# hmc-lair-shark-tracking/auv-sim

Hardware: AMD Instinct MI355X
Metric: RRT-Dubins node expansions/s (RRT.exploring) (higher is better)
Workload: dtype f64; 1 GPU; RRT.exploring 256 obst 200x200 cells 10000 iters x 12288 episodes/GPU, timebin parent sampling; episodes_per_gpu=12288, iters=10000, obstacles=256, cells=40000, parallelism=episodes sharded x1

## Files before the change

### auv_sim_amd/csrc/rrt_rows_body.h

```cpp
  extern __shared__ __align__(16) unsigned char smem[];
  const RrtTables S = rrt_tables_view(smem, W.n_habitats, W.n_poly);
  const int wave = (int)(threadIdx.x >> 6);
  const int lane = lane_id();
  const int row = lane >> 4, rl = lane & 15, rowbase = lane & 48;
  const int K = P.K;
  const int wg_waves = (int)(blockDim.x >> 6);
#if AUVP_ROWS_BODY_STREAM
  const RowsStreamLdsPlan plan = rrt_rows_stream_lds_plan(K, RW_MAX_OBST, rrt_tables_bytes(W.n_habitats, W.n_poly, W.n_bins), wg_waves, MIRROR);
  unsigned char* ebase = smem + plan.tables + (size_t)(wave * RW_ROWS + row) * plan.per_ep;
  double* ring = reinterpret_cast<double*>(ebase);
  double* inc = reinterpret_cast<double*>(ebase + plan.ring);
  uint16_t* bin_count = reinterpret_cast<uint16_t*>(ebase + plan.ring + plan.scratch);
#else
  const RowsLdsPlan plan = rrt_rows_lds_plan(K, RW_MAX_OBST, rrt_tables_bytes(W.n_habitats, W.n_poly, W.n_bins), wg_waves);
  unsigned char* ebase = smem + plan.tables + (size_t)(wave * RW_ROWS + row) * plan.per_ep;
  uint32_t* mt = reinterpret_cast<uint32_t*>(ebase);
  double* win = reinterpret_cast<double*>(ebase + plan.mt);
  double* inc = win;
  uint16_t* bin_count = reinterpret_cast<uint16_t*>(ebase + plan.mt + plan.scratch);
#endif

  rrt_tables_stage(S, W);
  if (threadIdx.x == 0) *S.params = P;
  const RrtParamsDev& Q = *S.params;
  double* olx = reinterpret_cast<double*>(smem + plan.tables + (size_t)wg_waves * RW_ROWS * plan.per_ep);
  double* oly = olx + RW_MAX_OBST;
  float* olr = reinterpret_cast<float*>(oly + RW_MAX_OBST);
  for (int i = threadIdx.x; i < RW_MAX_OBST; i += blockDim.x) { olx[i] = W.os_x[i]; oly[i] = W.os_y[i]; olr[i] = W.os_r[i]; }
  __syncthreads();

  const int ep = ((int)blockIdx.x * wg_waves + wave) * RW_ROWS + row;
  bool live = ep < n_episodes;
  const int eps = live ? ep : 0;
  if (!wave_any(live)) return;

  const int capn = B.cap_nodes, capp = B.cap_points, bcap = B.bin_cap;
  double* nodeF = B.node_f + (size_t)eps * capn * 8;
  int4* nodeI = reinterpret_cast<int4*>(B.node_i) + (size_t)eps * capn;
  uint8_t* nodeQ = B.node_q + (size_t)eps * capn;
  double* ptF = B.points + (size_t)eps * capp * 6;
  const BinLists bins = bin_lists(B, (size_t)eps, K);
  int next_chunk = 0;
  const double* init = B.init + (size_t)eps * 6;

#if AUVP_ROWS_BODY_STREAM
  RowStream rng;
  rng.ring = ring;
  rng.src = B.stream + (size_t)eps * (size_t)B.stream_cap;
  rng.pos = 0u; rng.front = 0u; rng.req = 0u;
  rng.cap = (uint32_t)B.stream_cap;
#pragma unroll
  for (int c = 0; c < RS_PEND; c++) rng.pend[c] = rs_piece(0.0);
#ifdef AUVP_STREAM_COUNT_SLOW
  rng.slow = 0u;
#endif
#define ROWS_CONSUME(on, n) stream_advance(rng, on, (uint32_t)(n))
#else
  RowRng rng;
  rng.s = mt;
  for (int i = rl; i < 624; i += 16) mt[i] = B.mt[(size_t)eps * 624 + i];
  {
    int idx = B.mt_index ? B.mt_index[eps] : 624;
    idx = idx < 0 ? 0 : (idx > 624 ? 624 : idx);
    rng.pslot = idx == 624 ? 0u : (uint32_t)idx;
    rng.avail = (uint32_t)(624 - idx);
    rng.drawn = 0ull;
  }
#define ROWS_CONSUME(on, n) rows_advance(rng, on, (uint32_t)(2 * (n)))
#endif
  for (int i = rl; i < K + 2; i += 16) bin_count[i] = 0;
  wave_sync();
  if (live && rl == 0) {
    nodeF[0] = init[0]; nodeF[1] = init[1]; nodeF[2] = init[2]; nodeF[3] = init[3]; nodeF[4] = init[5];
    nodeI[0] = make_int4(0, -1, 0, 0);
    nodeQ[0] = 0;
    bins.direct[(K >= 1 ? 1 : 0) * AUVP_BIN_HEAD] = 0;
    bin_count[K >= 1 ? 1 : 0] = 1;
  }
  wave_sync();
  int n_nodes = 1, n_points = 0, status = 0, n_cand = 0, iters_run = 0;
  const double4 sbox = reinterpret_cast<const double4*>(W.os_box)[rl];
  const int nv_poly = W.n_poly;

  for (int it = 0; it < P.max_iter; it++) {
    if (!wave_any(live)) break;
    int par = 0, n_total = 0, base = 0;
    {
      bool search = live;
      int fo = 0, rb = 0, cnt = 0;
      double u = 0.0;
#if AUVP_ROWS_BODY_STREAM
      StreamBase<MIRROR> sel;
#endif
      for (;;) {
#if AUVP_ROWS_BODY_STREAM
        if (!stream_ensure<MIRROR>(rng, search, 16u, rl) && search) { status = AUVP_ST_STREAM; live = false; iters_run = it; search = false; }
        sel = stream_base<MIRROR>(rng, 0u, rl);
        if (search) u = stream_read(sel, rl, rl);
#else
        rows_ensure(rng, search, 32u, rl);
        if (search) { u = rows_random_at(rng, (uint32_t)rl); win[rl] = u; }
#endif
        const int rbj = (int)py_uniform(1.0, (double)(K + 1), u);
        const bool cand = search && rl < 14;
        const bool badkey = cand && rbj > K;
        const int cj = (cand && !badkey) ? (int)bin_count[rbj] : 0;
        const uint32_t okm = row_ballot(cj != 0, rowbase), badm = row_ballot(badkey, rowbase);
        const int f_ok = okm ? (__ffs((int)okm) - 1) : 16, f_bad = badm ? (__ffs((int)badm) - 1) : 16;
        if (search) {
          if (f_bad < f_ok) { status = -5; live = false; iters_run = it; search = false; }
          else if (f_ok < 16) { fo = f_ok; search = false; }
        }
        const bool again = search;
        ROWS_CONSUME(again, 14);
        const int src = rowbase + (again ? 0 : fo);
        const int rb_n = row_read(rbj, src), cnt_n = row_read(cj, src);
        if (!again && live && cnt == 0) { rb = rb_n; cnt = cnt_n; }
        if (!wave_any(again)) break;
      }
#if AUVP_ROWS_BODY_STREAM
      const double u1 = stream_read(sel, fo + 1, rl), u2 = stream_read(sel, fo + 2, rl);
#else
      wave_sync();
      const double u1 = win[fo + 1], u2 = win[fo + 2];
#endif
      if (live) {
        const int ri = (int)py_uniform(0.0, (double)cnt, u1);
        par = bin_member(bins, rb, ri);
        n_total = (int)auvp_floor(py_uniform(0.0, Q.freq, u2) / 1);
        base = fo + 3;
      }
    }
    const bool on0 = live && 0 < n_total;
    const int n0_ = on0 ? (n_total < RW_C ? n_total : RW_C) : 0;
#if AUVP_ROWS_BODY_STREAM
    if (!stream_ensure<MIRROR>(rng, on0, (uint32_t)(base + 3 * n0_), rl) && on0) { status = AUVP_ST_STREAM; live = false; iters_run = it; }
#else
    auto make_window = [&](bool on, int nwin, int b0) {
      rows_ensure(rng, on, (uint32_t)(2 * (b0 + nwin)), rl);
#pragma unroll
      for (int t = 0; t < 3; t++) {
        const int j = rl + 16 * t;
        if (on && j < nwin) win[j] = rows_random_at(rng, (uint32_t)(b0 + j));
      }
      wave_sync();
    };
    {
      const int e_end = base + 3 * n0_;
      rows_ensure(rng, on0, (uint32_t)(2 * e_end), rl);
#pragma unroll
      for (int t = 0; t < 3; t++) {
        const int e = 16 + rl + 16 * t;
        if (on0 && e < e_end) win[e] = rows_random_at(rng, (uint32_t)e);
      }
      wave_sync();
    }
#endif
    double cx = 0.0, cy = 0.0, cth = 0.0, ctt = 0.0, clen = 0.0;
    if (live) {
      const double2 a = *reinterpret_cast<const double2*>(nodeF + (size_t)par * 8);
      const double2 b = *reinterpret_cast<const double2*>(nodeF + (size_t)par * 8 + 2);
      cx = a.x; cy = a.y; cth = b.x; ctt = b.y;
      clen = nodeF[(size_t)par * 8 + 4];
    }
#if AUVP_ROWS_BODY_STREAM
    stream_top_up<MIRROR>(rng, live, rl);
#endif
    const double px0 = cx, py0 = cy, clen0 = clen;
    int cnt = 0;
    double ptx[2] = {0.0, 0.0}, pty[2] = {0.0, 0.0};
    bool ptv[2] = {false, false};
    bool first_pass = true;
#pragma unroll
    for (int pass = 0; pass < 2; pass++) {
      const int c0 = pass * RW_C;
      const bool on = live && c0 < n_total;
      if (!wave_any(on)) break;
      const int n = on ? ((n_total - c0) < RW_C ? (n_total - c0) : RW_C) : 0;
      const int nwin = 3 * n;
#ifdef AUVP_ROWS_PAD
      {
        double pd0 = cth, pd1 = cx, pd2 = cy, pd3 = ctt;
#pragma unroll
        for (int q = 0; q < AUVP_ROWS_PAD / 4; q++)
          asm volatile("v_add_f64 %0, %0, 1.0\n\tv_add_f64 %1, %1, 1.0\n\tv_add_f64 %2, %2, 1.0\n\tv_add_f64 %3, %3, 1.0"
                       : "+v"(pd0), "+v"(pd1), "+v"(pd2), "+v"(pd3));
      }
#endif
      const int b0 = first_pass ? base : 0;
#if AUVP_ROWS_BODY_STREAM
      if (pass != 0 && !stream_ensure<MIRROR>(rng, on, (uint32_t)nwin, rl) && on) { status = AUVP_ST_STREAM; live = false; iters_run = it; }
      const StreamBase<MIRROR> wb = stream_base<MIRROR>(rng, (uint32_t)b0, rl);
#define ROWS_WIN(j) stream_read(wb, (j), rl)
#else
      if (pass != 0) make_window(on, nwin, b0);
      const double* wp = win + (pass == 0 ? base : 0);
#define ROWS_WIN(j) wp[j]
#endif
      unsigned long long tpred = 0ull;
#pragma unroll
      for (int t = 0; t < 3; t++) {
        const int j = rl + 16 * t;
        const double dist = py_uniform(0.0, Q.dist_to_end, ROWS_WIN(j));
        const double diff = py_uniform(-Q.diff_max, Q.diff_max, ROWS_WIN(j + 1));
        const unsigned long long fb = __builtin_amdgcn_fcmp(auvp_fabs(dist), auvp_fabs(diff), 2 ) &
                                      __builtin_amdgcn_uicmp((unsigned)(j + 1), (unsigned)nwin, 36 );
        tpred |= ((fb >> rowbase) & 0xffffull) << (16 * t);
      }
      const bool active = rl < n;
      const uint32_t mywin = active ? (uint32_t)(tpred >> (2 * rl)) : 0u;
      const uint32_t below_me = active ? ((1u << rl) - 1u) : 0u;
      int cbelow = active ? rl : 0;
      uint32_t tmask;
      for (;;) {
        const unsigned long long tb = __builtin_amdgcn_uicmp((mywin >> cbelow) & 1u, 0u, 33 );
        tmask = (uint32_t)((tb >> rowbase) & 0xffffull);
        const int cnew = __popc(tmask & below_me);
        const unsigned long long chg = __builtin_amdgcn_uicmp((unsigned)cnew, (unsigned)cbelow, 33 );
        cbelow = cnew;
        if (chg == 0ull) break;
      }
      const int mypos = 2 * rl + cbelow;
      const int used = 2 * n + __popc(tmask);
      const bool taken = (tmask >> rl) & 1u;
      double radius = 0.0, phi = 0.0, vt = 1.0;
      if (taken) {
        const double dist = py_uniform(0.0, Q.dist_to_end, ROWS_WIN(mypos));
        const double diff = py_uniform(-Q.diff_max, Q.diff_max, ROWS_WIN(mypos + 1));
        const double s1 = dist + diff, s2 = dist - diff;
        radius = auvp_div_plain(s1 + s2, -s1 + s2);
        phi = auvp_div_plain(s1 + s2, 2 * radius);
        vt = py_uniform(0.0, 2 * Q.v, ROWS_WIN(mypos + 2));
      }
#undef ROWS_WIN
#if !AUVP_ROWS_BODY_STREAM
      wave_sync();
#endif
      inc[rl] = phi;
      wave_sync();
      const double th = rows_theta_chain(cth, inc);
      const double myth = (rl == 15) ? cth : th;
      double sn, cs;
      auvp_sincos_sk(myth, &sn, &cs);
      double dx = 0.0, dy = 0.0, mv = 0.0, dt = 0.0;
      {
        const uint32_t below = tmask & ((1u << rl) - 1u);
        const int prev = below ? (31 - __clz((int)below)) : 15;
        const double so = row_read_f64(sn, rowbase + prev), co = row_read_f64(cs, rowbase + prev);
        if (taken) {
          dx = radius * (sn - so);
          dy = radius * (-cs + co);
          mv = auvp_sqrt_plain(dx * dx + dy * dy);
          dt = auvp_div_plain(mv, vt);
        }
      }
      if (rl < 15) { inc[rl] = dx; inc[18 + rl] = dy; inc[36 + rl] = dt; inc[54 + rl] = mv; }
      else { inc[15] = 0.0; inc[33] = 0.0; inc[51] = 0.0; inc[69] = 0.0; }
      wave_sync();
      if (rl < 4 && on) {
        double acc = rl == 0 ? cx : (rl == 1 ? cy : (rl == 2 ? ctt : clen));
        double2* rowp = reinterpret_cast<double2*>(inc + rl * 18);
        double2 v[8];
#pragma unroll
        for (int s2 = 0; s2 < 8; s2++) v[s2] = rowp[s2];
#pragma unroll
        for (int s2 = 0; s2 < 8; s2++) { acc = acc + v[s2].x; v[s2].x = acc; acc = acc + v[s2].y; v[s2].y = acc; }
#pragma unroll
        for (int s2 = 0; s2 < 8; s2++) rowp[s2] = v[s2];
      }
      wave_sync();
      double mx = 0.0, my = 0.0, mt_ = 0.0, ml = 0.0;
      if (active) { mx = inc[rl]; my = inc[18 + rl]; mt_ = inc[36 + rl]; ml = inc[54 + rl]; }
      const bool app = taken && (mv >= Q.min_dist);
      const uint32_t amask = row_ballot(app, rowbase);
      const int napp = __popc(amask);
      if (on && (n_points + cnt + napp > capp)) { status = -2; live = false; iters_run = it; }
      const bool wr = app && live;
      if (wr) {
        const int rank = __popc(amask & ((1u << rl) - 1u));
        const size_t gi = (size_t)(n_points + cnt + rank);
        double* ra = ptF + gi * 3;
        double* rb = ptF + (size_t)capp * 3 + gi * 3;
        typedef double nt_f64x2 __attribute__((ext_vector_type(2)));
        nt_f64x2 va, vb; va.x = mx; va.y = my; vb.x = myth; vb.y = vt;
        __builtin_nontemporal_store(va, reinterpret_cast<nt_f64x2*>(ra)); __builtin_nontemporal_store(mt_, ra + 2);
        __builtin_nontemporal_store(vb, reinterpret_cast<nt_f64x2*>(rb)); __builtin_nontemporal_store(ml, rb + 2);
      }
      ptx[pass] = mx; pty[pass] = my; ptv[pass] = wr;
      {
        const int last = n > 0 ? n - 1 : 0;
        const double th_last = row_read_f64(myth, rowbase + last);
        if (on) {
          cnt += napp;
          cx = inc[last]; cy = inc[18 + last]; ctt = inc[36 + last]; clen = inc[54 + last];
          cth = th_last;
        }
      }
      ROWS_CONSUME(on && live, b0 + used);
      first_pass = false;
      wave_sync();
    }
    ROWS_CONSUME(live && n_total == 0, base);

    const double reach = clen - clen0;
    const double bx0 = px0 - reach, by0 = py0 - reach, bx1 = px0 + reach, by1 = py0 + reach;
    const double slack = 0x1p-30 * (auvp_fabs(bx0) + auvp_fabs(bx1) + auvp_fabs(by0) + auvp_fabs(by1) + 1.0);
    const double hx = reach + slack;
    bool hit = false;
    double ex0 = bx0, ey0 = by0, ex1 = bx1, ey1 = by1;
    auto cull_and_test = [&](auto tight_tag) {
      constexpr bool TIGHT = decltype(tight_tag)::value;
      const double hs = hx + slack;
      const bool slot_hit = live && !(sbox.z < px0 - hs || sbox.x > px0 + hs || sbox.w < py0 - hs || sbox.y > py0 + hs);
      uint32_t sm = row_ballot(slot_hit, rowbase);
      double tcx = px0, tcy = py0, thx = hx, thy = hx;
      if (TIGHT) {
        double mnx = px0, mxx = px0, mny = py0, mxy = py0;
#pragma unroll
        for (int q = 0; q < 2; q++) {
          if (ptv[q]) {
            mnx = __builtin_fmin(mnx, ptx[q]); mxx = __builtin_fmax(mxx, ptx[q]);
            mny = __builtin_fmin(mny, pty[q]); mxy = __builtin_fmax(mxy, pty[q]);
          }
        }
        mnx = row_min_f64(mnx); mxx = row_max_f64(mxx); mny = row_min_f64(mny); mxy = row_max_f64(mxy);
        const double ts = 0x1p-30 * (auvp_fabs(mnx) + auvp_fabs(mxx) + auvp_fabs(mny) + auvp_fabs(mxy) + 1.0);
        tcx = (mnx + mxx) * 0.5; tcy = (mny + mxy) * 0.5;
        thx = (mxx - mnx) * 0.5 + ts; thy = (mxy - mny) * 0.5 + ts;
        const bool tight = slot_hit && !(sbox.z < mnx - ts || sbox.x > mxx + ts || sbox.w < mny - ts || sbox.y > mxy + ts);
        sm = row_ballot(tight, rowbase);
        ex0 = mnx; ey0 = mny; ex1 = mxx; ey1 = mxy;
      }
      while (wave_any(sm != 0u)) {
        const bool hs_ = sm != 0u;
        const int j0 = hs_ ? 16 * (__ffs((int)sm) - 1) : 0;
        sm &= sm - 1u;
        const int oi = j0 + rl;
        const double oxj = olx[oi], oyj = oly[oi], orj = (double)olr[oi];
        const double otj = W.os_t[oi];
        const bool cand = hs_ && (TIGHT ? !(auvp_fabs(oxj - tcx) > thx + orj || auvp_fabs(oyj - tcy) > thy + orj)
                                        : !(auvp_fabs(oxj - px0) > hx + orj || auvp_fabs(oyj - py0) > hx + orj));
        uint32_t cm = row_ballot(cand, rowbase);
        n_cand += __popc(cm);
        while (wave_any(cm != 0u)) {
          const bool has = cm != 0u;
          const int cl = has ? (__ffs((int)cm) - 1) : 0;
          cm &= cm - 1u;
          const double ox = row_read_f64(oxj, rowbase + cl), oy = row_read_f64(oyj, rowbase + cl), ot = row_read_f64(otj, rowbase + cl);
#pragma unroll
          for (int q = 0; q < 2; q++) {
            const double ddx = ptx[q] - ox, ddy = pty[q] - oy;
            hit |= has && ptv[q] && (ddx * ddx + ddy * ddy <= ot);
          }
          if (rl == 15) { const double ddx = px0 - ox, ddy = py0 - oy; hit |= has && (ddx * ddx + ddy * ddy <= ot); }
          if (row_ballot(hit, rowbase) != 0u) cm = 0u;
        }
      }
    };
    if (P.flags & AUVP_KFLAG_TIGHT_CULL) cull_and_test(std::true_type{});
    else cull_and_test(std::false_type{});
    const double* sb = S.world->safe_box;
    const bool box_inside = W.has_safe_box && ex0 > sb[0] && ey0 > sb[1] && ex1 < sb[2] && ey1 < sb[3];
    bool outside = false;
    if (wave_any(live && !box_inside)) {
      auto crossing_outside = [&](double x, double y) {
        if (nv_poly <= 0) return true;
        int par_ = 0;
        for (int e = 0; e < nv_poly; e++) {
          const int ej = e == 0 ? nv_poly - 1 : e - 1;
          const double xi = S.poly[e][0], yi = S.poly[e][1], xj = S.poly[ej][0], yj = S.poly[ej][1];
          if ((yi > y) != (yj > y)) par_ ^= (x < (xj - xi) * (y - yi) / (yj - yi) + xi) ? 1 : 0;
        }
        return (par_ & 1) == 0;
      };
      const bool need = live && !box_inside;
#pragma unroll
      for (int q = 0; q < 2; q++)
        if (need && ptv[q]) outside |= crossing_outside(ptx[q], pty[q]);
      if (need && rl == 15) outside |= crossing_outside(px0, py0);
    }
    const bool bad = row_ballot(hit || outside, rowbase) != 0u;
    const bool ok = live && !bad;
    if (ok && n_nodes >= capn) { status = -2; live = false; iters_run = it; }
    const bool acc_ = ok && live;
    const int me = n_nodes;
    if (acc_) {
      double q = auvp_floor(ctt * Q.inv_bin_interval);
      const double r = auvp_fma(-q, Q.bin_interval, ctt);
      if (r < 0.0) q -= 1.0;
      else if (r >= Q.bin_interval) q += 1.0;
      const double fi = q + 1.0;
      const double curr_bin = fi * Q.bin_interval;
      const bool over = curr_bin > Q.max_traj_time;
      bool stored = true;
      if (!over || fi <= (double)K) {
        const int bi = (int)fi;
        const int c = over ? 0 : (int)bin_count[bi];
        int32_t* slot = (c >= bcap || c >= 65535) ? nullptr : bin_slot_for_append(bins, bi, c, next_chunk, rl == 0);
        if (!slot) { status = -2; live = false; iters_run = it; stored = false; }
        else if (rl == 0) { *slot = me; bin_count[bi] = (uint16_t)(c + 1); }
      }
      if (stored) {
        if (rl == 0) {
          double* nf = nodeF + (size_t)me * 8;
          *reinterpret_cast<double2*>(nf) = make_double2(cx, cy);
          *reinterpret_cast<double2*>(nf + 2) = make_double2(cth, ctt);
          nf[4] = clen;
          nodeI[me] = make_int4(it, par, n_points, cnt);
          nodeQ[me] = ctt >= Q.max_traj_time - 30 ? 1 : 0;
        }
        n_nodes++;
        n_points += cnt;
      }
    }
    wave_sync();
  }

  const bool valid = ep < n_episodes;
  if (live) iters_run = P.max_iter;
#if AUVP_ROWS_BODY_STREAM
  const unsigned long long drawn = 2ull * rng.pos;
  if (!stream_ensure<MIRROR>(rng, valid && status == 0, 1u, rl) && valid && status == 0) status = AUVP_ST_STREAM;
  const double after = status == AUVP_ST_STREAM ? 0.0 : stream_read(stream_base<MIRROR>(rng, 0u, rl), rl, rl);
#else
  const unsigned long long drawn = rng.drawn;
  rows_ensure(rng, valid, 2u, rl);
  const double after = rows_random_at(rng, 0u);
#endif
  if (valid) {
    for (int i = rl; i < K + 1; i += 16) B.bin_count[(size_t)ep * (K + 1) + i] = (int32_t)bin_count[i];
    if (rl == 0) {
      RrtSummary& s = B.summary[ep];
#if AUVP_ROWS_BODY_STREAM
      pipe_report(B.pipe_fail, status == AUVP_ST_STREAM ? AUVP_ST_PIPELINE : 0);
#endif
      s.status = status; s.n_nodes = n_nodes; s.n_points = n_points; s.n_leaves = 0;
      s.best_leaf = -1; s.best_path_len = 0; s.iters_run = iters_run; s.n_candidates = n_cand;
      s.best_cost[0] = __builtin_inf(); s.best_cost[1] = 0.0; s.best_cost[2] = 0.0; s.best_cost[3] = 0.0;
      s.best_length = 0.0;
      s.rng_after = after; s.leaf_elems = 0; s.n_draw32 = drawn; s.nn_scanned = 0ull;
#if AUVP_ROWS_BODY_STREAM && defined(AUVP_STREAM_COUNT_SLOW)
      s.nn_scanned = rng.slow;
#endif
    }
  }
#undef ROWS_CONSUME
```

### auv_sim_amd/csrc/rrt_rows_stream_kernel.h

```cpp
#ifndef AUVP_RRT_ROWS_STREAM_KERNEL_H
#define AUVP_RRT_ROWS_STREAM_KERNEL_H
#include "rrt_rows_kernel.h"

namespace auvp {

constexpr int RS_RING = 256;
constexpr int RS_MIRROR = 48;
constexpr int RS_WAVES = 16;
#ifndef AUVP_RS_PIECE
#define AUVP_RS_PIECE 2
#endif
constexpr int RS_PIECE = AUVP_RS_PIECE;
constexpr int RS_CHUNK = 16 * RS_PIECE;
constexpr int RS_PEND = 64 / RS_CHUNK;
typedef double rs_f64x2 __attribute__((ext_vector_type(2)));
template <int N> struct RsPiece { typedef double type; };
template <> struct RsPiece<2> { typedef rs_f64x2 type; };
typedef RsPiece<RS_PIECE>::type rs_piece;
constexpr int RS_LDS_LIMIT = 160 * 1024;

struct RowsStreamLdsPlan {
  int tables, ring, scratch, bins, per_ep, obst, total;
};
__host__ __device__ inline RowsStreamLdsPlan rrt_rows_stream_lds_plan(int K, int n_obst_slots, int tables_bytes, int waves = RW_WAVES, bool mirror = false) {
  RowsStreamLdsPlan p;
  p.tables = (tables_bytes + 15) & ~15;
  p.ring = (RS_RING + (mirror ? RS_MIRROR : 0)) * 8;
  p.scratch = (4 * 18 * 8 + 15) & ~15;
  p.bins = (((K + 2) * 2) + 15) & ~15;
  p.per_ep = p.ring + p.scratch + p.bins;
  p.obst = n_obst_slots * (8 + 8 + 4);
  p.total = p.tables + waves * RW_ROWS * p.per_ep + p.obst;
  return p;
}

struct RowsStreamShape {
  int waves;
  bool mirror;
  RowsStreamLdsPlan plan;
};
__host__ inline RowsStreamShape rrt_rows_stream_shape(int K, int n_obst_slots, int tables_bytes, int waves_wanted, int force = -1) {
  int sw = waves_wanted < 1 ? 1 : (waves_wanted > RW_WAVES ? RW_WAVES : waves_wanted);
  while (sw > 1 && rrt_rows_stream_lds_plan(K, n_obst_slots, tables_bytes, sw, false).total > RS_LDS_LIMIT) sw--;
  bool mirror = force < 0 ? rrt_rows_stream_lds_plan(K, n_obst_slots, tables_bytes, sw, true).total <= RS_LDS_LIMIT : force != 0;
  while (mirror && sw > 1 && rrt_rows_stream_lds_plan(K, n_obst_slots, tables_bytes, sw, true).total > RS_LDS_LIMIT) sw--;
  RowsStreamShape s;
  s.waves = sw; s.mirror = mirror;
  s.plan = rrt_rows_stream_lds_plan(K, n_obst_slots, tables_bytes, sw, mirror);
  return s;
}

struct RowStream {
  double* ring;
  const double* src;
  uint32_t pos, front, req, cap;
  rs_piece pend[RS_PEND];
#ifdef AUVP_STREAM_COUNT_SLOW
  uint32_t slow;
#endif
};

template <bool MIRROR>
__device__ __forceinline__ void stream_commit(RowStream& r, int rl) {
#pragma unroll
  for (int c = 0; c < RS_PEND; c++)
    if (r.front + (uint32_t)(RS_CHUNK * c) < r.req) {
      const uint32_t s = (r.front + (uint32_t)(RS_CHUNK * c) + (uint32_t)(RS_PIECE * rl)) & (uint32_t)(RS_RING - 1);
      *reinterpret_cast<rs_piece*>(r.ring + s) = r.pend[c];
      if (MIRROR && s < (uint32_t)RS_MIRROR) *reinterpret_cast<rs_piece*>(r.ring + s + (uint32_t)RS_RING) = r.pend[c];
    }
  r.front = r.req;
}
__device__ __forceinline__ void stream_request(RowStream& r, bool on, int rl) {
  const uint32_t room = (uint32_t)RS_RING - (r.front - r.pos), left = r.cap - r.req;
  uint32_t n = (room < left ? room : left) / (uint32_t)RS_CHUNK;
  n = n > (uint32_t)RS_PEND ? (uint32_t)RS_PEND : n;
  n = on ? n : 0u;
#pragma unroll
  for (int c = 0; c < RS_PEND; c++)
    if ((uint32_t)c < n)
      r.pend[c] = __builtin_nontemporal_load(reinterpret_cast<const rs_piece*>(r.src + r.req + (uint32_t)(RS_CHUNK * c) + (uint32_t)(RS_PIECE * rl)));
  r.req += (uint32_t)RS_CHUNK * n;
}
template <bool MIRROR>
__device__ __forceinline__ void stream_top_up(RowStream& r, bool on, int rl) {
  stream_commit<MIRROR>(r, rl);
  stream_request(r, on, rl);
}
template <bool MIRROR>
__device__ __forceinline__ bool stream_ensure(RowStream& r, bool want, uint32_t need, int rl) {
  const uint32_t need_w = want ? need : 0u;
  const bool ok = r.pos + need_w <= r.cap;
  for (;;) {
    if (__builtin_amdgcn_uicmp(r.front - r.pos, ok ? need_w : 0u, 36 ) == 0ull) break;
    const bool go = ok && r.front - r.pos < need_w;
#ifdef AUVP_STREAM_COUNT_SLOW
    if (go) r.slow++;
#endif
    stream_commit<MIRROR>(r, rl);
    stream_request(r, go && ok, rl);
    stream_commit<MIRROR>(r, rl);
    wave_sync();
    if (!wave_any(go && ok && r.front - r.pos < need_w)) break;
  }
  wave_sync();
  return ok;
}
template <bool MIRROR> struct StreamBase;
template <> struct StreamBase<true> { const double* p; };
template <> struct StreamBase<false> { const double* ring; uint32_t first; };
template <bool MIRROR>
__device__ __forceinline__ StreamBase<MIRROR> stream_base(const RowStream& r, uint32_t b, int rl) {
  if constexpr (MIRROR) return StreamBase<true>{r.ring + (((r.pos + b) & (uint32_t)(RS_RING - 1)) + (uint32_t)rl)};
  else return StreamBase<false>{r.ring, r.pos + b};
}
__device__ __forceinline__ double stream_read(const StreamBase<true>& w, int j, int rl) { return w.p[j - rl]; }
__device__ __forceinline__ double stream_read(const StreamBase<false>& w, int j, int) { return w.ring[(w.first + (uint32_t)j) & (uint32_t)(RS_RING - 1)]; }
__device__ __forceinline__ void stream_advance(RowStream& r, bool on, uint32_t n) {
  if (on) r.pos += n;
}

template <int MAXW>
static __global__ __launch_bounds__(MAXW * 64, 1) void rrt_rows_stream_kernel(WorldDev W, RrtParamsDev P, RrtBuffers B, int n_episodes) {
  constexpr bool MIRROR = true;
#define AUVP_ROWS_BODY_STREAM 1
#include "rrt_rows_body.h"
#undef AUVP_ROWS_BODY_STREAM
}
template <int MAXW>
static __global__ __launch_bounds__(MAXW * 64, 1) void rrt_rows_stream_masked_kernel(WorldDev W, RrtParamsDev P, RrtBuffers B, int n_episodes) {
  constexpr bool MIRROR = false;
#define AUVP_ROWS_BODY_STREAM 1
#include "rrt_rows_body.h"
#undef AUVP_ROWS_BODY_STREAM
}

}
#endif
```

Before: 1.290 billion expansions/s.

## Fetch obstacle threshold via scalar constant loads per row instead of vector gather

```diff
diff --git a/auv_sim_amd/csrc/rrt_rows_body.h b/auv_sim_amd/csrc/rrt_rows_body.h
--- a/auv_sim_amd/csrc/rrt_rows_body.h
+++ b/auv_sim_amd/csrc/rrt_rows_body.h
@@ -79,7 +79,11 @@
   }
   wave_sync();
   int n_nodes = 1, n_points = 0, status = 0, n_cand = 0, iters_run = 0;
-  const double4 sbox = reinterpret_cast<const double4*>(W.os_box)[rl];
+  double4 sbox_ld = reinterpret_cast<const double4*>(W.os_box)[rl];
+  asm volatile("" : "+v"(sbox_ld.x), "+v"(sbox_ld.y), "+v"(sbox_ld.z), "+v"(sbox_ld.w));
+  const double4 sbox = sbox_ld;
+  typedef const __attribute__((address_space(4))) double* rows_ost_ptr;
+  const rows_ost_ptr ost_s = (rows_ost_ptr)W.os_t;
   const int nv_poly = W.n_poly;
 
   for (int it = 0; it < P.max_iter; it++) {
@@ -175,7 +179,7 @@
     for (int pass = 0; pass < 2; pass++) {
       const int c0 = pass * RW_C;
       const bool on = live && c0 < n_total;
-      if (!wave_any(on)) break;
+      if (pass != 0 && !wave_any(on)) break;
       const int n = on ? ((n_total - c0) < RW_C ? (n_total - c0) : RW_C) : 0;
       const int nwin = 3 * n;
 #ifdef AUVP_ROWS_PAD
@@ -337,7 +341,9 @@
         sm &= sm - 1u;
         const int oi = j0 + rl;
         const double oxj = olx[oi], oyj = oly[oi], orj = (double)olr[oi];
-        const double otj = W.os_t[oi];
+#ifdef AUVP_ROWS_OST_LDS
+        const double otj = orj * orj;
+#endif
         const bool cand = hs_ && (TIGHT ? !(auvp_fabs(oxj - tcx) > thx + orj || auvp_fabs(oyj - tcy) > thy + orj)
                                         : !(auvp_fabs(oxj - px0) > hx + orj || auvp_fabs(oyj - py0) > hx + orj));
         uint32_t cm = row_ballot(cand, rowbase);
@@ -346,7 +352,22 @@
           const bool has = cm != 0u;
           const int cl = has ? (__ffs((int)cm) - 1) : 0;
           cm &= cm - 1u;
-          const double ox = row_read_f64(oxj, rowbase + cl), oy = row_read_f64(oyj, rowbase + cl), ot = row_read_f64(otj, rowbase + cl);
+          const double ox = row_read_f64(oxj, rowbase + cl), oy = row_read_f64(oyj, rowbase + cl);
+#ifdef AUVP_ROWS_OST_LDS
+          const double ot = row_read_f64(otj, rowbase + cl);
+#else
+          const int oc = j0 + cl;
+          const unsigned long long hasm = __builtin_amdgcn_uicmp((unsigned)has, 0u, 33 );
+          double ot = 0.0;
+          int rowv = row;
+          asm volatile("" : "+v"(rowv));
+#pragma unroll
+          for (int r = 0; r < RW_ROWS; r++)
+            if (hasm & (1ull << (16 * r))) {
+              const double t = ost_s[__builtin_amdgcn_readlane(oc, 16 * r)];
+              ot = rowv == r ? t : ot;
+            }
+#endif
 #pragma unroll
           for (int q = 0; q < 2; q++) {
             const double ddx = ptx[q] - ox, ddy = pty[q] - oy;
diff --git a/auv_sim_amd/csrc/rrt_rows_stream_kernel.h b/auv_sim_amd/csrc/rrt_rows_stream_kernel.h
--- a/auv_sim_amd/csrc/rrt_rows_stream_kernel.h
+++ b/auv_sim_amd/csrc/rrt_rows_stream_kernel.h
@@ -82,6 +82,10 @@
       r.pend[c] = __builtin_nontemporal_load(reinterpret_cast<const rs_piece*>(r.src + r.req + (uint32_t)(RS_CHUNK * c) + (uint32_t)(RS_PIECE * rl)));
   r.req += (uint32_t)RS_CHUNK * n;
 }
+__device__ __forceinline__ void stream_settle(RowStream& r) {
+#pragma unroll
+  for (int c = 0; c < RS_PEND; c++) asm volatile("" : "+v"(r.pend[c]));
+}
 template <bool MIRROR>
 __device__ __forceinline__ void stream_top_up(RowStream& r, bool on, int rl) {
   stream_commit<MIRROR>(r, rl);
@@ -100,6 +104,7 @@
     stream_commit<MIRROR>(r, rl);
     stream_request(r, go && ok, rl);
     stream_commit<MIRROR>(r, rl);
+    stream_settle(r);
     wave_sync();
     if (!wave_any(go && ok && r.front - r.pos < need_w)) break;
   }
```

Result: faster. 1.368 billion expansions/s, median of 6 (+6.0%).
